# manonkok/Rao-Blackwellized-SLAM-smoothing

Hardware: AMD Instinct MI355X
Metric: particle-steps/s (filter) + smoother wall-clock, N=65k T=3k (higher is better)
Workload: dtype f64

## Files before the change

include/rbpf.h:

```cpp
#ifndef RBPF_H_
#define RBPF_H_

#include <stddef.h>
#include <stdint.h>

#ifdef __cplusplus
extern "C" {
#endif

#define RBPF_ABI_VERSION 9

typedef enum {
  RBPF_OK = 0,
  RBPF_ERR_INVALID_ARG = 1,
  RBPF_ERR_UNSUPPORTED = 2,
  RBPF_ERR_HIP = 3,
  RBPF_ERR_NO_DEVICE = 4,
  RBPF_ERR_OUT_OF_MEMORY = 5,
  RBPF_ERR_CHOL_FAILED = 6,
  RBPF_ERR_STATE = 7,
  RBPF_ERR_CALLBACK = 8
} rbpf_status;

typedef enum {
// ... 221 lines not shown

int rbpf_philox_fill(uint64_t seed, int32_t k_iter, int32_t N_P, int32_t N_T, int32_t n_w,
                     double* U, double* Z, double* Ufin);
int rbpf_meas_model(const rbpf_model* model, int32_t n_nonlin, int32_t n_pred, const double* xn,
                    double* dy);
int rbpf_dyn_model(const rbpf_model* model, int32_t n_nonlin, int32_t n_w, int32_t n_odo,
                   int32_t n_p, const double* xn, const double* odo, double dt, const double* Q,
                   const double* z, double* xn_next);
int rbpf_dyn_res_norm(const rbpf_model* model, int32_t n_nonlin, int32_t n_w, int32_t n_odo,
                      int32_t n_p, const double* xnk_t, const double* xn, const double* odo,
                      double dt, const double* Q, double* e_dyn);
int rbpf_sample(int32_t N, const double* w, int32_t n_draws, const double* u, int32_t* ind);
int rbpf_jacobian_phi3d(const rbpf_model* model, int32_t n_p, const double* x,
                        const double* lower, const double* upper, double* J);
int rbpf_chol_weights(int32_t M, int32_t batch, const double* S, const double* e, double jitter,
                      int32_t variant, int32_t reps, double* logw, int32_t* status, double* ms);
int32_t rbpf_chol_refresh_resolve(int32_t model_kind, int32_t n_lin, int32_t n_y, int32_t requested);
int rbpf_chol_sweep_probe(int32_t n, int32_t d, int32_t batch, const double* L, const double* U, const double* V,
                          const double* eta, int32_t reps, double* L_out, double* logw, int32_t* status, double* ms);
int rbpf_ext_pack_whiten_probe(int32_t dy_layout, int32_t rows, int32_t d, int32_t n, const double* dy_host,
                               const double* W_host, int32_t fused, double* G_host);
int rbpf_quat_helpers(int32_t op, int32_t n, const double* in, double* out);
int rbpf_probe_wave_reduce(const double* in, double* out);

typedef struct {
  int32_t struct_size;
  int32_t m_basis;
  const int32_t* NN;
  double L[3];
  const double* mean;
  const double* V;
  double sigma2;
  const double* var_table;
} rbpf_loc_map;

typedef struct {
  int32_t struct_size;
  int32_t N_P, N_T;
  int32_t x0_cols;
  int32_t q_pages;
  int32_t dt_len;
  int32_t odo_ld;
  const double* odometry;
  const double* y;
  const double* x0_nonlin;
  const double* Q;
// ... 71 lines not shown
```

rao-blackwellized-slam-smoothing_amd/_ffi.py:

```python
from __future__ import annotations

import ctypes as C
import importlib.util
import os
import sys

from . import _build

c_double_p = C.POINTER(C.c_double)
c_int32_p = C.POINTER(C.c_int32)

RBPF_OK = 0
RBPF_ERR_INVALID_ARG = 1
RBPF_ERR_UNSUPPORTED = 2
RBPF_ERR_HIP = 3
RBPF_ERR_NO_DEVICE = 4
RBPF_ERR_OUT_OF_MEMORY = 5
RBPF_ERR_CHOL_FAILED = 6
RBPF_ERR_STATE = 7
RBPF_ERR_CALLBACK = 8

RBPF_MODEL_DENSE_MAG_6D = 1
RBPF_MODEL_DENSE_RADIO_2DH = 2
RBPF_MODEL_SPARSE_VISUAL_2D = 3
# ... 100 lines not shown
class rbpf_ekf_problem(_SizedStructure):
    _fields_ = [("struct_size", C.c_int32), ("n_runs", C.c_int32), ("N_T", C.c_int32), ("q_pages", C.c_int32),
                ("dt_len", C.c_int32), ("odo_ld", C.c_int32), ("keep_P", C.c_int32), ("models", C.POINTER(C.POINTER(rbpf_model))),
                ("odometry", c_double_p), ("y", c_double_p), ("x0", c_double_p), ("q0", c_double_p), ("P0", c_double_p),
                ("R", c_double_p), ("LL", c_double_p), ("Q", c_double_p), ("dt", c_double_p)]


class rbpf_ekf_out(_SizedStructure):
    _fields_ = [("struct_size", C.c_int32), ("reserved", C.c_int32), ("xf_traj", c_double_p), ("qnb_traj", c_double_p),
                ("Pf", c_double_p)]


ABI_STRUCTS = [rbpf_model, rbpf_problem, rbpf_rng, rbpf_options, rbpf_filter_out, rbpf_smoother_out, rbpf_timing, rbpf_callbacks, rbpf_view,
               rbpf_loc_map, rbpf_loc_problem, rbpf_loc_out, rbpf_ekf_problem, rbpf_ekf_out]

EXPORTS = [
    "rbpf_abi_version", "rbpf_abi_sizeof", "rbpf_status_string", "rbpf_last_error", "rbpf_device_count", "rbpf_device_bytes_live",
    "rbpf_particle_filter", "rbpf_particle_smoother", "rbpf_particle_smoother_device",
    "rbpf_filter_create", "rbpf_filter_workspace_bytes", "rbpf_filter_advance", "rbpf_filter_reset", "rbpf_sync",
    "rbpf_filter_finish", "rbpf_filter_tell", "rbpf_filter_schedule", "rbpf_filter_one_launch_flushes", "rbpf_filter_resample_fallbacks", "rbpf_plan_refresh", "rbpf_chol_refresh_resolve", "rbpf_shard_smoother_refresh_reserve", "rbpf_shard_xn_traj", "rbpf_filter_ancestors", "rbpf_filter_step_external", "rbpf_filter_external_layout", "rbpf_filter_ancestors_device",
    "rbpf_filter_step_device", "rbpf_filter_set_device_callbacks",
    "rbpf_filter_sparse_gathered_device", "rbpf_filter_step_sparse_device", "rbpf_filter_sparse_yhattraj", "rbpf_timing_enable", "rbpf_timing_read", "rbpf_destroy",
    "rbpf_philox_fill", "rbpf_meas_model", "rbpf_dyn_model", "rbpf_dyn_res_norm", "rbpf_sample",
    "rbpf_jacobian_phi3d", "rbpf_chol_weights", "rbpf_chol_sweep_probe", "rbpf_ext_pack_whiten_probe", "rbpf_quat_helpers", "rbpf_probe_wave_reduce",
    "rbpf_shard_create", "rbpf_shard_views_get", "rbpf_shard_normalise_search", "rbpf_shard_pack", "rbpf_shard_step",
    "rbpf_shard_trajectories", "rbpf_shard_plan", "rbpf_shard_plan_read", "rbpf_shard_normalise_plan",
    "rbpf_stream_get", "rbpf_shard_set_async", "rbpf_shard_finish", "rbpf_shard_set_ancestors",
    "rbpf_shard_smoother_create", "rbpf_shard_smoother_views_get", "rbpf_shard_smoother_begin",
    "rbpf_shard_smoother_normalise", "rbpf_shard_smoother_anc_weights", "rbpf_shard_smoother_anc_sample",
    "rbpf_shard_smoother_refresh_begin", "rbpf_shard_smoother_refresh_pack", "rbpf_shard_smoother_refresh_end",
    "rbpf_shard_smoother_step", "rbpf_shard_smoother_end",
    "rbpf_particle_filter_localization", "rbpf_loc_create", "rbpf_loc_advance", "rbpf_loc_finish", "rbpf_loc_workspace_bytes",
    "rbpf_loc_predict", "rbpf_loc_dyn_model",
    "rbpf_loc_backward_simulate", "rbpf_loc_history", "rbpf_loc_backward_workspace_bytes", "rbpf_loc_backward_step",
    "rbpf_ekf_dense", "rbpf_ekf_workspace_bytes",
]

ABI_VERSION = 9
_lib = None


class RBPFError(RuntimeError):
    def __init__(self, status, msg):
        super().__init__(f"rbpf status {status}: {msg}")
        self.status = status


# ... 65 lines not shown
    lib.rbpf_filter_step_sparse_device.argtypes = [C.c_void_p, C.c_void_p, C.c_void_p, C.c_int32, C.c_void_p, C.c_int32]
    lib.rbpf_filter_sparse_yhattraj.argtypes = [C.c_void_p, c_double_p]
    lib.rbpf_stream_get.argtypes = [C.c_void_p, C.POINTER(C.c_void_p)]
    lib.rbpf_timing_enable.argtypes = [C.c_void_p, C.c_int32]
    lib.rbpf_timing_read.argtypes = [C.c_void_p, C.POINTER(rbpf_timing), C.c_int32]
    lib.rbpf_destroy.argtypes = [C.c_void_p]
    lib.rbpf_philox_fill.argtypes = [C.c_uint64, C.c_int32, C.c_int32, C.c_int32, C.c_int32, c_double_p, c_double_p,
                                     c_double_p]
    lib.rbpf_meas_model.argtypes = [C.POINTER(rbpf_model), C.c_int32, C.c_int32, c_double_p, c_double_p]
    lib.rbpf_dyn_model.argtypes = [C.POINTER(rbpf_model), C.c_int32, C.c_int32, C.c_int32, C.c_int32, c_double_p,
                                   c_double_p, C.c_double, c_double_p, c_double_p, c_double_p]
    lib.rbpf_dyn_res_norm.argtypes = [C.POINTER(rbpf_model), C.c_int32, C.c_int32, C.c_int32, C.c_int32, c_double_p,
                                      c_double_p, c_double_p, C.c_double, c_double_p, c_double_p]
    lib.rbpf_sample.argtypes = [C.c_int32, c_double_p, C.c_int32, c_double_p, c_int32_p]
    lib.rbpf_jacobian_phi3d.argtypes = [C.POINTER(rbpf_model), C.c_int32, c_double_p, c_double_p, c_double_p,
                                        c_double_p]
    lib.rbpf_chol_weights.argtypes = [C.c_int32, C.c_int32, c_double_p, c_double_p, C.c_double, C.c_int32, C.c_int32,
                                      c_double_p, c_int32_p, c_double_p]
    lib.rbpf_chol_sweep_probe.argtypes = [C.c_int32, C.c_int32, C.c_int32, c_double_p, c_double_p, c_double_p, c_double_p, C.c_int32,
                                          c_double_p, c_double_p, c_int32_p, c_double_p]
    lib.rbpf_ext_pack_whiten_probe.argtypes = [C.c_int32, C.c_int32, C.c_int32, C.c_int32, c_double_p, c_double_p, C.c_int32,
                                               c_double_p]
    lib.rbpf_quat_helpers.argtypes = [C.c_int32, C.c_int32, c_double_p, c_double_p]
    lib.rbpf_chol_refresh_resolve.argtypes = [C.c_int32, C.c_int32, C.c_int32, C.c_int32]
    lib.rbpf_chol_refresh_resolve.restype = C.c_int32
    lib.rbpf_particle_filter_localization.argtypes = [C.POINTER(rbpf_loc_map), C.POINTER(rbpf_loc_problem), C.POINTER(rbpf_rng),
                                                      C.POINTER(rbpf_options), C.POINTER(rbpf_loc_out)]
    lib.rbpf_loc_create.argtypes = [C.POINTER(rbpf_loc_map), C.POINTER(rbpf_loc_problem), C.POINTER(rbpf_rng),
                                    C.POINTER(rbpf_options), C.POINTER(C.c_void_p)]
    lib.rbpf_loc_advance.argtypes = [C.c_void_p, C.c_int32]
    lib.rbpf_loc_finish.argtypes = [C.c_void_p, C.POINTER(rbpf_loc_out)]
    lib.rbpf_loc_workspace_bytes.argtypes = [C.POINTER(rbpf_loc_map), C.POINTER(rbpf_loc_problem), C.POINTER(rbpf_options),
                                             C.POINTER(C.c_size_t)]
    lib.rbpf_loc_predict.argtypes = [C.POINTER(rbpf_loc_map), C.c_int32, c_double_p, c_double_p, c_double_p, C.c_int32, c_double_p]
    lib.rbpf_loc_dyn_model.argtypes = [C.c_int32, c_double_p, c_double_p, C.c_double, c_double_p, c_double_p, c_double_p]
    lib.rbpf_loc_backward_simulate.argtypes = [C.c_void_p, C.c_int32, c_double_p, C.c_uint64, c_double_p, c_int32_p, c_double_p]
    lib.rbpf_loc_history.argtypes = [C.c_void_p, c_double_p]
    lib.rbpf_loc_backward_workspace_bytes.argtypes = [C.c_int32, C.c_int32, C.c_int32, C.POINTER(C.c_size_t)]
    lib.rbpf_loc_backward_step.argtypes = [C.c_int32, C.c_int32, c_double_p, c_double_p, c_double_p, c_double_p, C.c_double, c_double_p,
                                           c_double_p, c_int32_p, c_double_p, C.c_int32, c_double_p]
    lib.rbpf_ekf_dense.argtypes = [C.POINTER(rbpf_ekf_problem), C.POINTER(rbpf_options), C.POINTER(rbpf_ekf_out)]
    lib.rbpf_ekf_workspace_bytes.argtypes = [C.POINTER(rbpf_ekf_problem), C.POINTER(rbpf_options), C.POINTER(C.c_size_t)]
    _lib = lib
    return lib


# ... 6 lines not shown
```

rao-blackwellized-slam-smoothing_amd/csrc/rbpf_api.hip:

```cpp
#include "../../include/rbpf.h"
#include "rbpf_internal.hpp"
#include "rbpf_ctx.hpp"
#include "rbpf_sparse.hpp"

#include <cmath>
#include <cstdio>
#include <cstdlib>
#include <cstring>
#include <string>
#include <vector>

namespace rbpf {

thread_local std::string g_last_error;

void set_error(const std::string& s) { g_last_error = s; }

int hip_fail(hipError_t e, const char* what, const char* file, int line) {
  char buf[512];
  snprintf(buf, sizeof(buf), "%s failed: %s (%s:%d)", what, hipGetErrorString(e), file, line);
  g_last_error = buf;
  (void)hipGetLastError();
  return (e == hipErrorOutOfMemory) ? RBPF_ERR_OUT_OF_MEMORY : RBPF_ERR_HIP;
}
// ... 334 lines not shown
  c->lazy_depth = (!sparse && c->opt.lazy_depth >= 2) ? std::min(c->opt.lazy_depth, smoother ? 3 : ((c->lay.sym && c->lay.CH64 == 8 && !c->fp32) ? (int)kMaxSets : (int)kMaxSetsFull)) : 1;
  {
    const bool can = !ex && c->lazy_depth >= 2 && (!smoother || c->opt.inplace > 0);
    if (c->opt.inplace > 0 && !can) { set_error("inplace=1 needs lazy_depth >= 2 and an unsharded session"); return RBPF_ERR_UNSUPPORTED; }
    c->inplace = c->opt.inplace > 0;
    if (c->opt.inplace == 0 && can) {
      size_t fr = 0, tot = 0;
      HIPCHK(hipMemGetInfo(&fr, &tot));
      const size_t two = 2 * c->bank_cap * (L.szT + L.szB) * (c->fp32 ? sizeof(float) : sizeof(double));
      c->inplace = (double)two > 0.85 * (double)fr;
    }
  }
  for (int b = 0; b < 2; ++b) {
    if (b == 1 && c->inplace) { c->Pt[1] = c->Pt[0]; c->Pb[1] = c->Pb[0]; }
    else {
      RB_TRY(c->pool.alloc(&c->Pt[b], c->fp32 ? (c->bank_cap * L.szT + 1) / 2 : c->bank_cap * L.szT));
      RB_TRY(c->pool.alloc(&c->Pb[b], c->fp32 ? (c->bank_cap * L.szB + 1) / 2 : c->bank_cap * L.szB));
    }
    RB_TRY(c->pool.alloc(&c->F[b], c->bank_cap * 2 * d * L.ldx));
    RB_TRY(c->pool.alloc(&c->xl[b], c->bank_cap * L.ldx));
    HIPCHK(hipMemsetAsync(c->F[b], 0, c->bank_cap * 2 * d * L.ldx * sizeof(double), c->stream));
    HIPCHK(hipMemsetAsync(c->xl[b], 0, c->bank_cap * L.ldx * sizeof(double), c->stream));
  }
  if (c->inplace) RB_TRY(c->pool.alloc(&c->d_ip, (size_t)8 * N));
  c->share_inplace = c->inplace && c->lazy_depth >= 2 && !ex && layout_shares_flush(c->lay);
  if (const char* e = tuning_env("RBPF_SHARE_INPLACE")) c->share_inplace = c->share_inplace && atoi(e) != 0;
  if (c->share_inplace) {
    RB_TRY(c->pool.alloc(&c->d_share_writers, 1));
    HIPCHK(hipMemset(c->d_share_writers, 0, sizeof(unsigned long long)));
  }
  c->share_flush = c->lazy_depth >= 2 && !c->inplace && !ex && layout_shares_flush(c->lay);
  if (const size_t sd = sym_strip_doubles(c->lay, d + (smoother ? 1 : 0))) {
    RB_TRY(c->pool.alloc(&c->d_strip_ws, (size_t)N * sd));
    c->strip_ws_stride = sd;
  }
  if (c->share_flush) {
    RB_TRY(c->pool.alloc(&c->d_share, (size_t)3 * N));
    RB_TRY(c->pool.alloc(&c->d_share_writers, 1));
    HIPCHK(hipMemset(c->d_share_writers, 0, sizeof(unsigned long long)));
  }
  if (c->lazy_depth >= 2) {
    if (!L.sym && (L.CH < 1 || L.CPL < 1 || L.CPL > 2)) { set_error("lazy_depth >= 2 needs 128 <= nLin with at most two row chunks per wave (full-square storage; block-lower storage, options.storage = 2, takes nLin 384..511)"); return RBPF_ERR_UNSUPPORTED; }
    if (!L.sym && step_lds_bytes(c->mdl, c->lay, smoother ? 1 : 0, c->lazy_depth) > 160 * 1024) { set_error("lazy_depth too large for the LDS plan"); return RBPF_ERR_UNSUPPORTED; }
    if (L.sym && step_sym_lds_bytes(c->mdl, c->lay, c->lazy_depth, 1, smoother ? 1 : 0) > 160 * 1024) { set_error("lazy_depth too large for the LDS plan"); return RBPF_ERR_UNSUPPORTED; }
    for (int b = 0; b <= c->lazy_depth; ++b) {
      RB_TRY(c->pool.alloc(&c->Fb[b], (size_t)(N + 1) * 2 * d * L.ldx));
      HIPCHK(hipMemsetAsync(c->Fb[b], 0, (size_t)(N + 1) * 2 * d * L.ldx * sizeof(double), c->stream));
// ... 1204 lines not shown
int rbpf_quat_helpers(int32_t op, int32_t n, const double* in, double* out) {
  if (!have_device()) { set_error("no HIP device"); return RBPF_ERR_NO_DEVICE; }
  if (op < 0 || op > 8 || n < 1 || !in || !out) { set_error("bad argument"); return RBPF_ERR_INVALID_ARG; }
  static const int nin_of[9] = {3, 3, 4, 4, 4, 4, 4, 4, 3}, nout_of[9] = {4, 4, 3, 3, 16, 16, 4, 9, 9};
  DevicePool tmp; double *di = nullptr, *dout = nullptr;
  RB_TRY(tmp.upload(&di, in, (size_t)n * nin_of[op])); RB_TRY(tmp.alloc(&dout, (size_t)n * nout_of[op]));
  HIPCHK(launch_quat_helpers(op, n, di, dout, 0));
  HIPCHK(hipDeviceSynchronize());
  HIPCHK(hipMemcpy(out, dout, (size_t)n * nout_of[op] * 8, hipMemcpyDeviceToHost));
  return RBPF_OK;
}

int rbpf_probe_wave_reduce(const double* in, double* out) {
  if (!have_device()) { set_error("no HIP device"); return RBPF_ERR_NO_DEVICE; }
  if (!in || !out) { set_error("bad argument"); return RBPF_ERR_INVALID_ARG; }
  DevicePool tmp; double *di = nullptr, *dout = nullptr;
  RB_TRY(tmp.upload(&di, in, 256)); RB_TRY(tmp.alloc(&dout, 4));
  HIPCHK(launch_probe_wave_reduce(di, dout, 0));
  HIPCHK(hipDeviceSynchronize());
  HIPCHK(hipMemcpy(out, dout, 4 * 8, hipMemcpyDeviceToHost));
  return RBPF_OK;
}

int rbpf_jacobian_phi3d(const rbpf_model* model, int32_t n_p, const double* x, const double* lower, const double* upper, double* J) {
  if (!have_device()) { set_error("no HIP device"); return RBPF_ERR_NO_DEVICE; }
  if (!model || model->kind != RBPF_MODEL_DENSE_MAG_6D || !x || !lower || !upper || !J || n_p < 1) { set_error("bad argument"); return RBPF_ERR_INVALID_ARG; }
  ModelDev M; DevicePool tmp; double *dx = nullptr, *dlo = nullptr, *dup = nullptr, *dj = nullptr;
  RB_TRY(model_for_helpers(model, 7, 6, 7, M, tmp));
  RB_TRY(tmp.upload(&dx, x, (size_t)3 * n_p)); RB_TRY(tmp.upload(&dlo, lower, 3)); RB_TRY(tmp.upload(&dup, upper, 3)); RB_TRY(tmp.alloc(&dj, (size_t)9 * M.m * n_p));
  HIPCHK(launch_jacobian_phi3d(M, n_p, dx, dlo, dup, dj, 0));
  HIPCHK(hipDeviceSynchronize());
  HIPCHK(hipMemcpy(J, dj, (size_t)9 * M.m * n_p * 8, hipMemcpyDeviceToHost));
  return RBPF_OK;
}

}
```

rao-blackwellized-slam-smoothing_amd/csrc/rbpf_internal.hpp:

```cpp
#pragma once
#include <hip/hip_runtime.h>
#include <stdint.h>
#include <stddef.h>
#include <stdlib.h>
#include <atomic>

namespace rbpf {

inline hipError_t lds_opt_in(const void* kernel, int bytes, std::atomic<uint64_t>& done) {
  int dev = 0;
  hipError_t e = hipGetDevice(&dev);
  if (e != hipSuccess) return e;
  const uint64_t bit = 1ull << (dev & 63);
  if (dev < 64 && (done.load(std::memory_order_acquire) & bit)) return hipSuccess;
  e = hipFuncSetAttribute(kernel, hipFuncAttributeMaxDynamicSharedMemorySize, bytes);
  if (e != hipSuccess) return e;
  if (dev < 64) done.fetch_or(bit, std::memory_order_release);
  return hipSuccess;
}

#ifdef RBPF_TUNING
inline const char* tuning_env(const char* key) { return getenv(key); }
#else
inline const char* tuning_env(const char*) { return nullptr; }
// ... 115 lines not shown
  const double* xn;
  double* traj_max;
  double* traj_mean;
  int* iw_max;
  double* lse_out;
  int parallel_scan = 0;
};

struct SearchArgs {
  int N, n_draw, t;
  int slot0 = 0;
  int u_is_scalar = 0;
  const double* wc;
  int rng_mode; int k_iter;
  const double* U;
  unsigned long long seed;
  int* ai;
  int* overflow;
  int scan_depth = 0;
  int approx = 0;
  int* ambiguous = nullptr;
  const double* w = nullptr;
  double* wc_exact = nullptr;
};

size_t step_lds_bytes(const ModelDev& m, const Layout& lay, int extra = 0, int n_sets = 1);
bool step_use_blocked(const ModelDev& m, const Layout& lay, int extra, int n_sets);
Layout make_layout(int n, int d);
Layout make_layout_low_regs(int n, int d);
Layout make_layout_sym(int n, int d, int fp32 = 0);
bool sym_supported(int n, int d);
size_t sym_strip_doubles(const Layout& lay, int d);
size_t step_sym_lds_bytes(const ModelDev& m, const Layout& lay, int n_sets, int write_base, int extra = 0);
hipError_t launch_step_sym(const StepArgs& a, hipStream_t s);
bool step_sym_shared_one_launch(const StepArgs& a);
hipError_t launch_step_sym_shared(const StepArgs& a, hipStream_t s);
hipError_t launch_probe_wave_reduce(const double* in, double* out, hipStream_t s);

hipError_t launch_propagate(const StepArgs& a, hipStream_t s);
hipError_t launch_step(const StepArgs& a, hipStream_t s);
hipError_t launch_step_wide_d2(const StepArgs& a, hipStream_t s);
hipError_t launch_step_wide_d4(const StepArgs& a, hipStream_t s);
hipError_t launch_step_wide_d5(const StepArgs& a, hipStream_t s);
hipError_t launch_step_wide_d6(const StepArgs& a, hipStream_t s);
hipError_t launch_step_wide_d7(const StepArgs& a, hipStream_t s);
hipError_t launch_step_wide_d8(const StepArgs& a, hipStream_t s);
hipError_t launch_normalise_scan(const NormArgs& a, hipStream_t s);
hipError_t launch_search(const SearchArgs& a, hipStream_t s);
hipError_t launch_cumsum(int N, const double* w, double* wc, hipStream_t s);
hipError_t launch_normalise_resample(const NormArgs& a, const SearchArgs& sa, int* order, int* counts, hipStream_t s,
                                     const int* remap = nullptr);
hipError_t launch_order_large(int n_slots, int range, const int* key, const int* remap, int* order, int* counts, hipStream_t s);
hipError_t launch_order(int n_slots, int range, const int* key, int* order, int* counts, hipStream_t s, const int* remap = nullptr);
hipError_t launch_inplace_plan(int N, const int* order, const int* ai, const int* base, int* dst, int* phase,
                               int* scratch, hipStream_t s);
hipError_t launch_share_inplace_plan(int N, const int* order, const int* ai, const int* base, int* dst, int* phase, int* scratch,
                                     unsigned long long* writers, hipStream_t s);
hipError_t launch_share_plan(int N, int nkeys, const int* ai, int* lead, int* dst, int* phase, unsigned long long* writers, hipStream_t s);
size_t resample_scratch_doubles(int N);
hipError_t launch_resample_pipeline(const NormArgs& nm, const SearchArgs* sa, int* order, int* counts, const int* remap,
                                    double* scratch, hipStream_t s);
hipError_t launch_resample_lse(int N, const double* scratch, double* out, hipStream_t s);
constexpr int kMaxParticles = 1024 * 1024;
constexpr int kSingleWgResampleMaxN = 8192;
hipError_t launch_resample_fixup(const SearchArgs& a, hipStream_t s);

hipError_t launch_pack_P(const Layout& lay, const double* P_colmajor, size_t src_stride, double* Pt,
                         double* Pb, int count, hipStream_t s, int fp32 = 0);
hipError_t launch_unpack_P(const Layout& lay, int d, const double* Pt, const double* Pb, const double* F,
                           const int* index, int count, double* P_colmajor, hipStream_t s, int fp32 = 0);
hipError_t launch_unpack_P_sets(const Layout& lay, int d, const double* Pt, const double* Pb, int n_sets,
                                const double* const* fset, const int* const* fidx, const int* base, const int* index,
                                int count, double* P_colmajor, hipStream_t s, int fp32 = 0);
hipError_t launch_weighted_mean_xl(int N, int n, int ldx, const double* xl, const double* w, double* out,
// ... 35 lines not shown
```

rao-blackwellized-slam-smoothing_amd/csrc/rbpf_kernels.hip:

```cpp
#include "rbpf_internal.hpp"
#include "rbpf_device.hpp"
#include "rbpf_model_dev.hpp"

#include <cstdlib>

#include "rbpf_step_full.hpp"

namespace rbpf {

Layout make_layout_low_regs(int n, int d) {
  Layout L = make_layout(n, d);
  if (L.CH == 2) { L.RS = 2; L.CS = 2; L.CPL = L.CH / L.RS; }
  return L;
}

#ifndef RBPF_KB_THRESHOLD_KB
#define RBPF_KB_THRESHOLD_KB 72
#endif
bool step_use_blocked(const ModelDev& m, const Layout& lay, int extra, int n_sets) {
  if (n_sets < 1 || lay.mc == 0 || lay.CPL < 1 || lay.CPL > 2 || lay.CH != lay.CPL * lay.RS || lay.RS * lay.CS != kWaves) return false;
  return (size_t)lds_plan(lay.n, m.d, extra, n_sets, lay.ldx, lay.CS, lay.mc, m.ktot, 0).total * sizeof(double) > (size_t)RBPF_KB_THRESHOLD_KB * 1024;
}

size_t step_lds_bytes(const ModelDev& m, const Layout& lay, int extra, int n_sets) {
// ... 521 lines not shown
}

hipError_t launch_order(int n_slots, int range, const int* key, int* order, int* counts, hipStream_t s, const int* remap) {
  if (range > kSingleWgResampleMaxN) return launch_order_large(n_slots, range, key, remap, order, counts, s);
  hipLaunchKernelGGL(order_kernel, dim3(1), dim3(kNormThreads), 0, s, n_slots, range, key, order, counts, remap);
  return hipGetLastError();
}

__global__ __launch_bounds__(kNormThreads) void cumsum_kernel(int N, const double* __restrict__ w,
                                                              double* __restrict__ wc) {
  __shared__ double sbuf[kScanChunk];
  __shared__ double sbuf2[kScanChunk];
  __shared__ double scarry;
  strict_cumsum_block(N, w, wc, sbuf, sbuf2, &scarry);
}

hipError_t launch_cumsum(int N, const double* w, double* wc, hipStream_t s) {
  hipLaunchKernelGGL(cumsum_kernel, dim3(1), dim3(kNormThreads), 0, s, N, w, wc);
  return hipGetLastError();
}

__global__ void search_kernel(const SearchArgs a) {
  const int i0 = blockIdx.x * blockDim.x + threadIdx.x;
  if (i0 >= a.n_draw) return;
  const int i = a.slot0 + i0;
  const double u = (a.rng_mode == 0) ? a.U[a.u_is_scalar ? 0 : i] : philox_resample_uniform(a.seed, i, a.t, a.k_iter);
  int lo = 0, hi = a.N;
  while (lo < hi) {
    const int mid = (lo + hi) >> 1;
    if (a.wc[mid] < u) lo = mid + 1; else hi = mid;
  }
  if (a.approx) {
    const double S = a.scan_depth > 0 ? (double)a.scan_depth : (double)((a.N + kNormThreads - 1) / kNormThreads) + 32.0;
    bool amb = false;
    if (lo < a.N) { const double p = a.wc[lo]; amb |= fabs(p - u) <= 1.7e-16 * ((double)lo + S) * fabs(p); }
    if (lo > 0) { const double p = a.wc[lo - 1]; amb |= fabs(p - u) <= 1.7e-16 * ((double)lo + S) * fabs(p); }
    if (amb) atomicAdd(a.ambiguous, 1);
  }
  if (lo >= a.N) { lo = a.N - 1; if (a.overflow) atomicAdd(a.overflow, 1); }
  a.ai[i] = lo;
}

__global__ __launch_bounds__(kNormThreads) void resample_fixup_kernel(const SearchArgs a) {
  __shared__ double sbuf[kScanChunk];
  __shared__ double sbuf2[kScanChunk];
  __shared__ double scarry;
// ... 479 lines not shown
```

rao-blackwellized-slam-smoothing_amd/csrc/rbpf_resample.hip:

```cpp
#include "rbpf_internal.hpp"
#include "rbpf_device.hpp"

namespace rbpf {

constexpr int kRB = 1024;

__device__ inline double blk_sum(double v, double* sred) {
  const int lane = threadIdx.x & 63, wave = threadIdx.x >> 6;
  v = wave_sum(v);
  __syncthreads();
  if (lane == 0) sred[wave] = v;
  __syncthreads();
  double s = sred[0];
  for (int w = 1; w < kRB / 64; ++w) s += sred[w];
  return s;
}

__device__ inline double blk_max(double v, double* sred) {
  const int lane = threadIdx.x & 63, wave = threadIdx.x >> 6;
#pragma unroll
  for (int off = 32; off > 0; off >>= 1) v = fmax(v, __shfl_xor(v, off, 64));
  __syncthreads();
  if (lane == 0) sred[wave] = v;
  __syncthreads();
  double s = sred[0];
  for (int w = 1; w < kRB / 64; ++w) s = fmax(s, sred[w]);
  return s;
}

__global__ __launch_bounds__(kRB) void rs_max_kernel(int N, const double* __restrict__ logw, double* __restrict__ pmax) {
  __shared__ double sred[16];
  const int i = blockIdx.x * kRB + threadIdx.x;
  const double m = blk_max(i < N ? logw[i] : -INFINITY, sred);
  if (threadIdx.x == 0) pmax[blockIdx.x] = m;
}

__device__ inline double global_max(const double* pmax, int B, double* sred) {
  double m = -INFINITY;
  for (int b = threadIdx.x; b < B; b += kRB) m = fmax(m, pmax[b]);
  return blk_max(m, sred);
}

__global__ __launch_bounds__(kRB) void rs_sumexp_kernel(int N, int B, const double* __restrict__ logw,
                                                        const double* __restrict__ pmax, double* __restrict__ psum) {
  __shared__ double sred[16];
  const double c = global_max(pmax, B, sred);
  const int i = blockIdx.x * kRB + threadIdx.x;
  const double s = blk_sum(i < N ? exp(logw[i] - c) : 0.0, sred);
  if (threadIdx.x == 0) psum[blockIdx.x] = s;
}

__global__ __launch_bounds__(kRB) void rs_weights_kernel(NormArgs a, int B, const double* __restrict__ pmax,
                                                         const double* __restrict__ psum, double* __restrict__ btot,
                                                         double* __restrict__ bparts ) {
  __shared__ double sred[16];
  __shared__ int sidx[16];
  __shared__ double sbc;
  const int tid = threadIdx.x, lane = tid & 63, wave = tid >> 6, N = a.N;
  const double c = global_max(pmax, B, sred);
  if (tid == 0) { double t = 0.0; for (int b = 0; b < B; ++b) t += psum[b]; sbc = c + log(t); }
  __syncthreads();
  const double lse = sbc;
  const int i = blockIdx.x * kRB + tid;
  const double wi = (i < N) ? exp(a.logw[i] - lse) : 0.0;
  if (i < N) a.w[i] = wi;
  double bw = (i < N) ? wi : -1.0;
  int bi = (i < N) ? i : 0x7fffffff;
#pragma unroll
  for (int off = 32; off > 0; off >>= 1) {
    const double ow = __shfl_xor(bw, off, 64);
    const int oi = __shfl_xor(bi, off, 64);
    if (ow > bw || (ow == bw && oi < bi)) { bw = ow; bi = oi; }
  }
  __syncthreads();
  if (lane == 0) { sred[wave] = bw; sidx[wave] = bi; }
  __syncthreads();
  if (tid == 0) {
    double gw = sred[0]; int gi = sidx[0];
    for (int w = 1; w < kRB / 64; ++w) if (sred[w] > gw || (sred[w] == gw && sidx[w] < gi)) { gw = sred[w]; gi = sidx[w]; }
    bparts[blockIdx.x * 10 + 0] = gw;
    bparts[blockIdx.x * 10 + 1] = (double)gi;
  }
  for (int cix = 0; cix < a.nN; ++cix) {
// ... 11 lines not shown
  __syncthreads();
  double woff = 0.0;
  for (int w = 0; w < wave; ++w) woff += sred[w];
  const double lp = woff + inc;
  if (i < N) a.wc[i] = lp;
  if (tid == kRB - 1) btot[blockIdx.x] = lp;
}

__global__ __launch_bounds__(kRB) void rs_offsets_kernel(NormArgs a, int B, const double* __restrict__ btot,
                                                         const double* __restrict__ bparts) {
  __shared__ double sb[1024];
  __shared__ double sp[16][10];
  __shared__ double soff;
  const int tid = threadIdx.x, N = a.N;
  for (int b = tid; b < B; b += kRB) sb[b] = btot[b];
  __syncthreads();
  if (tid == 0) { double t = 0.0; for (int b = 0; b < (int)blockIdx.x; ++b) t += sb[b]; soff = t; }
  __syncthreads();
  const int i = blockIdx.x * kRB + tid;
  if (i < N && blockIdx.x > 0) a.wc[i] = soff + a.wc[i];
  if (blockIdx.x == 0) {
    if (tid < 2 + a.nN) {
      const int q = tid;
      if (q >= 2) {
        double t = 0.0;
        for (int b = 0; b < B; ++b) t += bparts[b * 10 + q];
        sp[0][q] = t;
      }
    }
    if (tid == 0) {
      double gw = bparts[0]; int gi = (int)bparts[1];
      for (int b = 1; b < B; ++b) { const double w = bparts[b * 10]; const int ix = (int)bparts[b * 10 + 1]; if (w > gw || (w == gw && ix < gi)) { gw = w; gi = ix; } }
      if (gi < 0 || gi >= N) gi = 0;
      *a.iw_max = gi;
      sp[1][0] = (double)gi;
    }
    __syncthreads();
    if (tid >= 2 && tid < 2 + a.nN) {
      const int cix = tid - 2, gi = (int)sp[1][0];
      if (a.traj_mean) a.traj_mean[cix] = sp[0][tid];
      if (a.traj_max) a.traj_max[cix] = a.xn[(size_t)cix * N + gi];
    }
  }
}

__global__ void rs_hist_kernel(int N, const int* __restrict__ key, const int* __restrict__ remap, int* __restrict__ counts) {
  const int i = blockIdx.x * blockDim.x + threadIdx.x;
  if (i < N) atomicAdd(&counts[remap ? remap[key[i]] : key[i]], 1);
}

__global__ __launch_bounds__(kRB) void rs_scan_kernel(int N, int* __restrict__ counts) {
  __shared__ int swave[kRB / 64];
  const int tid = threadIdx.x, lane = tid & 63, wave = tid >> 6;
  const int S = (N + kRB - 1) / kRB;
  const int j0 = min(tid * S, N), j1 = min(j0 + S, N);
  constexpr int NBATCH = 8;
  int tot = 0;
  for (int jb = j0; jb < j1; jb += NBATCH) {
    int v[NBATCH];
#pragma unroll
    for (int k = 0; k < NBATCH; ++k) v[k] = counts[min(jb + k, N - 1)];
#pragma unroll
    for (int k = 0; k < NBATCH; ++k) tot += (jb + k < j1) ? v[k] : 0;
  }
  int inc = tot;
#pragma unroll
  for (int off = 1; off < 64; off <<= 1) { const int o = __shfl_up(inc, off, 64); if (lane >= off) inc += o; }
  if (lane == 63) swave[wave] = inc;
  __syncthreads();
  int run = inc - tot;
  for (int w = 0; w < wave; ++w) run += swave[w];
  for (int jb = j0; jb < j1; jb += NBATCH) {
    int v[NBATCH];
#pragma unroll
    for (int k = 0; k < NBATCH; ++k) v[k] = counts[min(jb + k, N - 1)];
#pragma unroll
    for (int k = 0; k < NBATCH; ++k)
      if (jb + k < j1) { counts[jb + k] = run; run += v[k]; }
  }
}

__global__ void rs_scatter_kernel(int N, const int* __restrict__ key, const int* __restrict__ remap, int* __restrict__ counts,
                                  int* __restrict__ order) {
  const int i = blockIdx.x * blockDim.x + threadIdx.x;
  if (i < N) order[atomicAdd(&counts[remap ? remap[key[i]] : key[i]], 1)] = i;
}

size_t resample_scratch_doubles(int N) { return (size_t)13 * ((N + kRB - 1) / kRB) + 16; }

hipError_t launch_resample_pipeline(const NormArgs& nm, const SearchArgs* sa, int* order, int* counts, const int* remap,
                                    double* scratch, hipStream_t s) {
  const int N = nm.N, B = (N + kRB - 1) / kRB;
  double* pmax = scratch; double* psum = pmax + B; double* btot = psum + B; double* bparts = btot + B;
  hipLaunchKernelGGL(rs_max_kernel, dim3(B), dim3(kRB), 0, s, N, nm.logw, pmax);
  hipLaunchKernelGGL(rs_sumexp_kernel, dim3(B), dim3(kRB), 0, s, N, B, nm.logw, pmax, psum);
  hipLaunchKernelGGL(rs_weights_kernel, dim3(B), dim3(kRB), 0, s, nm, B, pmax, psum, btot, bparts);
  hipLaunchKernelGGL(rs_offsets_kernel, dim3(B), dim3(kRB), 0, s, nm, B, btot, bparts);
  hipError_t e = hipGetLastError();
  if (e != hipSuccess || !sa) return e;
  SearchArgs q = *sa;
  q.scan_depth = B + 32;
  if ((e = launch_search(q, s)) != hipSuccess) return e;
  if (q.approx && (e = launch_resample_fixup(q, s)) != hipSuccess) return e;
  if (order) {
    if ((e = hipMemsetAsync(counts, 0, (size_t)N * sizeof(int), s)) != hipSuccess) return e;
    const int nb = (q.n_draw + 255) / 256;
    hipLaunchKernelGGL(rs_hist_kernel, dim3(nb), dim3(256), 0, s, q.n_draw, q.ai, remap, counts);
    hipLaunchKernelGGL(rs_scan_kernel, dim3(1), dim3(kRB), 0, s, N, counts);
    hipLaunchKernelGGL(rs_scatter_kernel, dim3(nb), dim3(256), 0, s, q.n_draw, q.ai, remap, counts, order);
    e = hipGetLastError();
  }
  return e;
}

__global__ void rs_lse_kernel(int B, const double* __restrict__ pmax, const double* __restrict__ psum, double* __restrict__ out) {
  double c = -INFINITY, t = 0.0;
  for (int b = 0; b < B; ++b) c = fmax(c, pmax[b]);
  for (int b = 0; b < B; ++b) t += psum[b];
  *out = c + log(t);
}

hipError_t launch_resample_lse(int N, const double* scratch, double* out, hipStream_t s) {
  const int B = (N + kRB - 1) / kRB;
  hipLaunchKernelGGL(rs_lse_kernel, dim3(1), dim3(1), 0, s, B, scratch, scratch + B, out);
  return hipGetLastError();
}

hipError_t launch_order_large(int n_slots, int range, const int* key, const int* remap, int* order, int* counts, hipStream_t s) {
  hipError_t e = hipMemsetAsync(counts, 0, (size_t)range * sizeof(int), s);
  if (e != hipSuccess) return e;
  const int nb = (n_slots + 255) / 256;
  hipLaunchKernelGGL(rs_hist_kernel, dim3(nb), dim3(256), 0, s, n_slots, key, remap, counts);
  hipLaunchKernelGGL(rs_scan_kernel, dim3(1), dim3(kRB), 0, s, range, counts);
  hipLaunchKernelGGL(rs_scatter_kernel, dim3(nb), dim3(256), 0, s, n_slots, key, remap, counts, order);
  return hipGetLastError();
}

__global__ void ip_mark_kernel(int N, const int* __restrict__ ai, const int* __restrict__ base, int* __restrict__ has,
                               int* __restrict__ nzp) {
  const int i = blockIdx.x * blockDim.x + threadIdx.x;
  if (i < N) { const int s = base[ai[i]]; has[s] = 1; nzp[s] = 1; }
}

__global__ void ip_free_kernel(int N, const int* __restrict__ has, const int* __restrict__ nzp, int* __restrict__ freelist) {
  const int f = blockIdx.x * blockDim.x + threadIdx.x;
  if (f < N && !has[f]) freelist[f - nzp[f]] = f;
}

__global__ void ip_assign_kernel(int N, const int* __restrict__ order, const int* __restrict__ ai, const int* __restrict__ base,
                                 const int* __restrict__ nzp, const int* __restrict__ freelist, int* __restrict__ dst,
                                 int* __restrict__ phase) {
  const int b = blockIdx.x * blockDim.x + threadIdx.x;
  if (b >= N) return;
  const int i = order[b];
  const int s = base[ai[i]];
  const int prev = (b > 0) ? base[ai[order[b - 1]]] : -1;
  const bool first = (s != prev);
  dst[i] = first ? s : freelist[b - nzp[s] - 1];
// ... 53 lines not shown
  const int b = blockIdx.x * blockDim.x + threadIdx.x;
  bool w = false;
  if (b < N) {
    const int i = order[b];
    w = lead[ai[i]] == i;
    if (w) {
      const int s = base[ai[i]];
      const bool first = leadbase[s] == b;
      dst[i] = first ? s : freelist[rank[b]];
      phase[i] = first ? 2 : 1;
    }
  }
  const unsigned long long m = __ballot(w);
  if (writers && (threadIdx.x & 63) == 0 && m) atomicAdd(writers, (unsigned long long)__popcll(m));
}
__global__ void sip_readers_kernel(int N, const int* __restrict__ ai, const int* __restrict__ lead, int* __restrict__ dst, int* __restrict__ phase) {
  const int i = blockIdx.x * blockDim.x + threadIdx.x;
  if (i < N && lead[ai[i]] != i) { dst[i] = dst[lead[ai[i]]]; phase[i] = 0; }
}

hipError_t launch_share_inplace_plan(int N, const int* order, const int* ai, const int* base, int* dst, int* phase, int* scratch,
                                     unsigned long long* writers, hipStream_t s) {
  int* lead = scratch; int* leadbase = scratch + N; int* has = scratch + 2 * (size_t)N; int* nzp = scratch + 3 * (size_t)N;
  int* freelist = scratch + 4 * (size_t)N; int* flag = scratch + 5 * (size_t)N;
  const int nb = (N + 255) / 256;
  hipLaunchKernelGGL(sip_fill_kernel, dim3(nb), dim3(256), 0, s, N, lead, leadbase, has, nzp);
  hipLaunchKernelGGL(sip_mark_kernel, dim3(nb), dim3(256), 0, s, N, ai, base, lead, has, nzp);
  hipLaunchKernelGGL(rs_scan_kernel, dim3(1), dim3(kRB), 0, s, N, nzp);
  hipLaunchKernelGGL(ip_free_kernel, dim3(nb), dim3(256), 0, s, N, has, nzp, freelist);
  hipLaunchKernelGGL(sip_first_kernel, dim3(nb), dim3(256), 0, s, N, order, ai, base, lead, leadbase);
  hipLaunchKernelGGL(sip_flag_kernel, dim3(nb), dim3(256), 0, s, N, order, ai, base, lead, leadbase, flag);
  hipLaunchKernelGGL(rs_scan_kernel, dim3(1), dim3(kRB), 0, s, N, flag);
  hipLaunchKernelGGL(sip_writers_kernel, dim3(nb), dim3(256), 0, s, N, order, ai, base, lead, leadbase, flag, freelist, dst, phase, writers);
  hipLaunchKernelGGL(sip_readers_kernel, dim3(nb), dim3(256), 0, s, N, ai, lead, dst, phase);
  return hipGetLastError();
}

hipError_t launch_inplace_plan(int N, const int* order, const int* ai, const int* base, int* dst, int* phase, int* scratch,
                               hipStream_t s) {
  int* has = scratch; int* nzp = scratch + N; int* freelist = scratch + 2 * (size_t)N;
  hipError_t e = hipMemsetAsync(scratch, 0, (size_t)2 * N * sizeof(int), s);
  if (e != hipSuccess) return e;
  const int nb = (N + 255) / 256;
  hipLaunchKernelGGL(ip_mark_kernel, dim3(nb), dim3(256), 0, s, N, ai, base, has, nzp);
  hipLaunchKernelGGL(rs_scan_kernel, dim3(1), dim3(kRB), 0, s, N, nzp);
  hipLaunchKernelGGL(ip_free_kernel, dim3(nb), dim3(256), 0, s, N, has, nzp, freelist);
  hipLaunchKernelGGL(ip_assign_kernel, dim3(nb), dim3(256), 0, s, N, order, ai, base, nzp, freelist, dst, phase);
  return hipGetLastError();
}

}
```

Before: 5.949 million.

## Replace single-block integer scans with multi-block scan in resample ordering

Swaps the single-workgroup serial-chunk exclusive scan used in counting-sort ordering and in-place plan building for a multi-block scan. Each block scans its own slice, and block offsets are then folded in, either by a separate add pass or directly inside the scatter kernel. The counts memset is folded into the search kernel, and the tid-0 serial reductions over block partials are batched so loads can be issued ahead of the adds. This is meant to remove a one-block serial bottleneck at N=65k, at the cost of extra launches, per-block recomputation of offsets, and a larger scratch buffer.

Result: no change. 5.928 million (-0.4%).

```diff
diff --git a/include/rbpf.h b/include/rbpf.h
--- a/include/rbpf.h
+++ b/include/rbpf.h
@@ -267,6 +267,8 @@
                                const double* W_host, int32_t fused, double* G_host);
 int rbpf_quat_helpers(int32_t op, int32_t n, const double* in, double* out);
 int rbpf_probe_wave_reduce(const double* in, double* out);
+int rbpf_order_scan_probe(int32_t n_slots, int32_t range, const int32_t* key, int32_t n_remap, const int32_t* remap, int32_t* order,
+                          int32_t* scan);
 
 typedef struct {
   int32_t struct_size;
diff --git a/rao-blackwellized-slam-smoothing_amd/_ffi.py b/rao-blackwellized-slam-smoothing_amd/_ffi.py
--- a/rao-blackwellized-slam-smoothing_amd/_ffi.py
+++ b/rao-blackwellized-slam-smoothing_amd/_ffi.py
@@ -146,7 +146,7 @@
     "rbpf_filter_step_device", "rbpf_filter_set_device_callbacks",
     "rbpf_filter_sparse_gathered_device", "rbpf_filter_step_sparse_device", "rbpf_filter_sparse_yhattraj", "rbpf_timing_enable", "rbpf_timing_read", "rbpf_destroy",
     "rbpf_philox_fill", "rbpf_meas_model", "rbpf_dyn_model", "rbpf_dyn_res_norm", "rbpf_sample",
-    "rbpf_jacobian_phi3d", "rbpf_chol_weights", "rbpf_chol_sweep_probe", "rbpf_ext_pack_whiten_probe", "rbpf_quat_helpers", "rbpf_probe_wave_reduce",
+    "rbpf_jacobian_phi3d", "rbpf_chol_weights", "rbpf_chol_sweep_probe", "rbpf_ext_pack_whiten_probe", "rbpf_quat_helpers", "rbpf_probe_wave_reduce", "rbpf_order_scan_probe",
     "rbpf_shard_create", "rbpf_shard_views_get", "rbpf_shard_normalise_search", "rbpf_shard_pack", "rbpf_shard_step",
     "rbpf_shard_trajectories", "rbpf_shard_plan", "rbpf_shard_plan_read", "rbpf_shard_normalise_plan",
     "rbpf_stream_get", "rbpf_shard_set_async", "rbpf_shard_finish", "rbpf_shard_set_ancestors",
@@ -258,6 +258,7 @@
     lib.rbpf_ext_pack_whiten_probe.argtypes = [C.c_int32, C.c_int32, C.c_int32, C.c_int32, c_double_p, c_double_p, C.c_int32,
                                                c_double_p]
     lib.rbpf_quat_helpers.argtypes = [C.c_int32, C.c_int32, c_double_p, c_double_p]
+    lib.rbpf_order_scan_probe.argtypes = [C.c_int32, C.c_int32, c_int32_p, C.c_int32, c_int32_p, c_int32_p, c_int32_p]
     lib.rbpf_chol_refresh_resolve.argtypes = [C.c_int32, C.c_int32, C.c_int32, C.c_int32]
     lib.rbpf_chol_refresh_resolve.restype = C.c_int32
     lib.rbpf_particle_filter_localization.argtypes = [C.POINTER(rbpf_loc_map), C.POINTER(rbpf_loc_problem), C.POINTER(rbpf_rng),
diff --git a/rao-blackwellized-slam-smoothing_amd/csrc/rbpf_api.hip b/rao-blackwellized-slam-smoothing_amd/csrc/rbpf_api.hip
--- a/rao-blackwellized-slam-smoothing_amd/csrc/rbpf_api.hip
+++ b/rao-blackwellized-slam-smoothing_amd/csrc/rbpf_api.hip
@@ -380,7 +380,7 @@
     HIPCHK(hipMemsetAsync(c->F[b], 0, c->bank_cap * 2 * d * L.ldx * sizeof(double), c->stream));
     HIPCHK(hipMemsetAsync(c->xl[b], 0, c->bank_cap * L.ldx * sizeof(double), c->stream));
   }
-  if (c->inplace) RB_TRY(c->pool.alloc(&c->d_ip, (size_t)8 * N));
+  if (c->inplace) RB_TRY(c->pool.alloc(&c->d_ip, (size_t)8 * N + scan_scratch_ints((size_t)N)));
   c->share_inplace = c->inplace && c->lazy_depth >= 2 && !ex && layout_shares_flush(c->lay);
   if (const char* e = tuning_env("RBPF_SHARE_INPLACE")) c->share_inplace = c->share_inplace && atoi(e) != 0;
   if (c->share_inplace) {
@@ -1631,6 +1631,31 @@
   return RBPF_OK;
 }
 
+int rbpf_order_scan_probe(int32_t n_slots, int32_t range, const int32_t* key, int32_t n_remap, const int32_t* remap, int32_t* order,
+                          int32_t* scan) {
+  if (!have_device()) { set_error("no HIP device"); return RBPF_ERR_NO_DEVICE; }
+  if (range < 1 || range > kMaxParticles || (!key && !scan) || (key && (!order || n_slots < 1 || n_slots > kMaxParticles)) ||
+      (remap && n_remap < 1)) { set_error("bad argument"); return RBPF_ERR_INVALID_ARG; }
+  const int nkeys = remap ? n_remap : range;
+  for (int i = 0; key && i < n_slots; ++i)
+    if (key[i] < 0 || key[i] >= nkeys || (remap && (remap[key[i]] < 0 || remap[key[i]] >= range))) { set_error("key out of range"); return RBPF_ERR_INVALID_ARG; }
+  DevicePool tmp; int *dkey = nullptr, *dremap = nullptr, *dorder = nullptr, *dcounts = nullptr, *dscan = nullptr, *dtot = nullptr;
+  if (key) {
+    RB_TRY(tmp.upload(&dkey, key, (size_t)n_slots)); RB_TRY(tmp.alloc(&dorder, (size_t)n_slots));
+    if (remap) RB_TRY(tmp.upload(&dremap, remap, (size_t)n_remap));
+    RB_TRY(tmp.alloc(&dcounts, (size_t)range + scan_scratch_ints((size_t)range)));
+    HIPCHK(launch_order_large(n_slots, range, dkey, dremap, dorder, dcounts, 0));
+  }
+  if (scan) {
+    RB_TRY(tmp.upload(&dscan, scan, (size_t)range)); RB_TRY(tmp.alloc(&dtot, scan_scratch_ints((size_t)range)));
+    HIPCHK(launch_scan_ints(range, dscan, dtot, 0));
+  }
+  HIPCHK(hipDeviceSynchronize());
+  if (key) HIPCHK(hipMemcpy(order, dorder, (size_t)n_slots * 4, hipMemcpyDeviceToHost));
+  if (scan) HIPCHK(hipMemcpy(scan, dscan, (size_t)range * 4, hipMemcpyDeviceToHost));
+  return RBPF_OK;
+}
+
 int rbpf_jacobian_phi3d(const rbpf_model* model, int32_t n_p, const double* x, const double* lower, const double* upper, double* J) {
   if (!have_device()) { set_error("no HIP device"); return RBPF_ERR_NO_DEVICE; }
   if (!model || model->kind != RBPF_MODEL_DENSE_MAG_6D || !x || !lower || !upper || !J || n_p < 1) { set_error("bad argument"); return RBPF_ERR_INVALID_ARG; }
diff --git a/rao-blackwellized-slam-smoothing_amd/csrc/rbpf_internal.hpp b/rao-blackwellized-slam-smoothing_amd/csrc/rbpf_internal.hpp
--- a/rao-blackwellized-slam-smoothing_amd/csrc/rbpf_internal.hpp
+++ b/rao-blackwellized-slam-smoothing_amd/csrc/rbpf_internal.hpp
@@ -161,6 +161,8 @@
   int* ambiguous = nullptr;
   const double* w = nullptr;
   double* wc_exact = nullptr;
+  int* zero = nullptr;
+  int n_zero = 0;
 };
 
 size_t step_lds_bytes(const ModelDev& m, const Layout& lay, int extra = 0, int n_sets = 1);
@@ -189,6 +191,8 @@
 hipError_t launch_cumsum(int N, const double* w, double* wc, hipStream_t s);
 hipError_t launch_normalise_resample(const NormArgs& a, const SearchArgs& sa, int* order, int* counts, hipStream_t s,
                                      const int* remap = nullptr);
+constexpr size_t scan_scratch_ints(size_t n) { return (n + 1023) / 1024; }
+hipError_t launch_scan_ints(int n, int* data, int* btot, hipStream_t s);
 hipError_t launch_order_large(int n_slots, int range, const int* key, const int* remap, int* order, int* counts, hipStream_t s);
 hipError_t launch_order(int n_slots, int range, const int* key, int* order, int* counts, hipStream_t s, const int* remap = nullptr);
 hipError_t launch_inplace_plan(int N, const int* order, const int* ai, const int* base, int* dst, int* phase,
diff --git a/rao-blackwellized-slam-smoothing_amd/csrc/rbpf_kernels.hip b/rao-blackwellized-slam-smoothing_amd/csrc/rbpf_kernels.hip
--- a/rao-blackwellized-slam-smoothing_amd/csrc/rbpf_kernels.hip
+++ b/rao-blackwellized-slam-smoothing_amd/csrc/rbpf_kernels.hip
@@ -567,6 +567,8 @@
 
 __global__ void search_kernel(const SearchArgs a) {
   const int i0 = blockIdx.x * blockDim.x + threadIdx.x;
+  if (a.zero)
+    for (int j = i0; j < a.n_zero; j += gridDim.x * blockDim.x) a.zero[j] = 0;
   if (i0 >= a.n_draw) return;
   const int i = a.slot0 + i0;
   const double u = (a.rng_mode == 0) ? a.U[a.u_is_scalar ? 0 : i] : philox_resample_uniform(a.seed, i, a.t, a.k_iter);
diff --git a/rao-blackwellized-slam-smoothing_amd/csrc/rbpf_resample.hip b/rao-blackwellized-slam-smoothing_amd/csrc/rbpf_resample.hip
--- a/rao-blackwellized-slam-smoothing_amd/csrc/rbpf_resample.hip
+++ b/rao-blackwellized-slam-smoothing_amd/csrc/rbpf_resample.hip
@@ -14,6 +14,19 @@
   double s = sred[0];
   for (int w = 1; w < kRB / 64; ++w) s += sred[w];
   return s;
+}
+
+constexpr int kSumBatch = 16;
+__device__ inline double ordered_sum(const double* __restrict__ x, int n, int stride) {
+  double t = 0.0;
+  for (int b0 = 0; b0 < n; b0 += kSumBatch) {
+    double v[kSumBatch];
+#pragma unroll
+    for (int k = 0; k < kSumBatch; ++k) v[k] = x[(size_t)min(b0 + k, n - 1) * stride];
+#pragma unroll
+    for (int k = 0; k < kSumBatch; ++k) if (b0 + k < n) t += v[k];
+  }
+  return t;
 }
 
 __device__ inline double blk_max(double v, double* sred) {
@@ -58,7 +71,7 @@
   __shared__ double sbc;
   const int tid = threadIdx.x, lane = tid & 63, wave = tid >> 6, N = a.N;
   const double c = global_max(pmax, B, sred);
-  if (tid == 0) { double t = 0.0; for (int b = 0; b < B; ++b) t += psum[b]; sbc = c + log(t); }
+  if (tid == 0) sbc = c + log(ordered_sum(psum, B, 1));
   __syncthreads();
   const double lse = sbc;
   const int i = blockIdx.x * kRB + tid;
@@ -116,15 +129,20 @@
   if (blockIdx.x == 0) {
     if (tid < 2 + a.nN) {
       const int q = tid;
-      if (q >= 2) {
-        double t = 0.0;
-        for (int b = 0; b < B; ++b) t += bparts[b * 10 + q];
-        sp[0][q] = t;
-      }
+      if (q >= 2) sp[0][q] = ordered_sum(bparts + q, B, 10);
     }
     if (tid == 0) {
       double gw = bparts[0]; int gi = (int)bparts[1];
-      for (int b = 1; b < B; ++b) { const double w = bparts[b * 10]; const int ix = (int)bparts[b * 10 + 1]; if (w > gw || (w == gw && ix < gi)) { gw = w; gi = ix; } }
+      for (int b0 = 1; b0 < B; b0 += kSumBatch) {
+        double vw[kSumBatch], vi[kSumBatch];
+#pragma unroll
+        for (int k = 0; k < kSumBatch; ++k) { const int b = min(b0 + k, B - 1); vw[k] = bparts[b * 10]; vi[k] = bparts[b * 10 + 1]; }
+#pragma unroll
+        for (int k = 0; k < kSumBatch; ++k) {
+          const double w = vw[k]; const int ix = (int)vi[k];
+          if (b0 + k < B && (w > gw || (w == gw && ix < gi))) { gw = w; gi = ix; }
+        }
+      }
       if (gi < 0 || gi >= N) gi = 0;
       *a.iw_max = gi;
       sp[1][0] = (double)gi;
@@ -138,46 +156,85 @@
   }
 }
 
-__global__ void rs_hist_kernel(int N, const int* __restrict__ key, const int* __restrict__ remap, int* __restrict__ counts) {
-  const int i = blockIdx.x * blockDim.x + threadIdx.x;
-  if (i < N) atomicAdd(&counts[remap ? remap[key[i]] : key[i]], 1);
-}
-
-__global__ __launch_bounds__(kRB) void rs_scan_kernel(int N, int* __restrict__ counts) {
+constexpr int kMaxScanBlocks = kMaxParticles / kRB;
+
+__global__ __launch_bounds__(kRB) void rs_blockscan_kernel(int n, int* __restrict__ data, int* __restrict__ btot) {
   __shared__ int swave[kRB / 64];
   const int tid = threadIdx.x, lane = tid & 63, wave = tid >> 6;
-  const int S = (N + kRB - 1) / kRB;
-  const int j0 = min(tid * S, N), j1 = min(j0 + S, N);
-  constexpr int NBATCH = 8;
-  int tot = 0;
-  for (int jb = j0; jb < j1; jb += NBATCH) {
-    int v[NBATCH];
-#pragma unroll
-    for (int k = 0; k < NBATCH; ++k) v[k] = counts[min(jb + k, N - 1)];
-#pragma unroll
-    for (int k = 0; k < NBATCH; ++k) tot += (jb + k < j1) ? v[k] : 0;
-  }
-  int inc = tot;
+  const int i = blockIdx.x * kRB + tid;
+  const int v = (i < n) ? data[i] : 0;
+  int inc = v;
 #pragma unroll
   for (int off = 1; off < 64; off <<= 1) { const int o = __shfl_up(inc, off, 64); if (lane >= off) inc += o; }
   if (lane == 63) swave[wave] = inc;
   __syncthreads();
-  int run = inc - tot;
+  int run = inc - v;
   for (int w = 0; w < wave; ++w) run += swave[w];
-  for (int jb = j0; jb < j1; jb += NBATCH) {
-    int v[NBATCH];
-#pragma unroll
-    for (int k = 0; k < NBATCH; ++k) v[k] = counts[min(jb + k, N - 1)];
-#pragma unroll
-    for (int k = 0; k < NBATCH; ++k)
-      if (jb + k < j1) { counts[jb + k] = run; run += v[k]; }
-  }
-}
-
-__global__ void rs_scatter_kernel(int N, const int* __restrict__ key, const int* __restrict__ remap, int* __restrict__ counts,
-                                  int* __restrict__ order) {
-  const int i = blockIdx.x * blockDim.x + threadIdx.x;
-  if (i < N) order[atomicAdd(&counts[remap ? remap[key[i]] : key[i]], 1)] = i;
+  if (i < n) data[i] = run;
+  if (tid == kRB - 1) btot[blockIdx.x] = run + v;
+}
+
+__device__ inline void rs_block_offsets(int B, const int* __restrict__ btot, int* sboff, int* swave) {
+  const int tid = threadIdx.x, lane = tid & 63, wave = tid >> 6, nwaves = blockDim.x >> 6;
+  int carry = 0;
+  for (int b0 = 0; b0 < B; b0 += blockDim.x) {
+    const int b = b0 + tid;
+    const int v = (b < B) ? btot[b] : 0;
+    int inc = v;
+#pragma unroll
+    for (int off = 1; off < 64; off <<= 1) { const int o = __shfl_up(inc, off, 64); if (lane >= off) inc += o; }
+    __syncthreads();
+    if (lane == 63) swave[wave] = inc;
+    __syncthreads();
+    int run = carry + inc - v;
+    for (int w = 0; w < wave; ++w) run += swave[w];
+    if (b < B) sboff[b] = run;
+    for (int w = 0; w < nwaves; ++w) carry += swave[w];
+  }
+  __syncthreads();
+}
+
+__global__ __launch_bounds__(kRB) void rs_addoffsets_kernel(int n, int B, int* __restrict__ data, const int* __restrict__ btot) {
+  __shared__ int sboff[kMaxScanBlocks];
+  __shared__ int swave[kRB / 64];
+  rs_block_offsets(B, btot, sboff, swave);
+  const int i = blockIdx.x * kRB + threadIdx.x;
+  if (i < n) data[i] += sboff[blockIdx.x];
+}
+
+hipError_t launch_scan_ints(int n, int* data, int* btot, hipStream_t s) {
+  const int B = (n + kRB - 1) / kRB;
+  if (n < 1 || B > kMaxScanBlocks) return hipErrorInvalidValue;
+  hipLaunchKernelGGL(rs_blockscan_kernel, dim3(B), dim3(kRB), 0, s, n, data, btot);
+  if (B > 1) hipLaunchKernelGGL(rs_addoffsets_kernel, dim3(B), dim3(kRB), 0, s, n, B, data, btot);
+  return hipGetLastError();
+}
+
+__global__ void rs_hist_kernel(int N, const int* __restrict__ key, const int* __restrict__ remap, int* __restrict__ counts) {
+  const int i = blockIdx.x * blockDim.x + threadIdx.x;
+  if (i < N) atomicAdd(&counts[remap ? remap[key[i]] : key[i]], 1);
+}
+
+__global__ __launch_bounds__(256) void rs_scatter_kernel(int N, int B, const int* __restrict__ key, const int* __restrict__ remap,
+                                                         int* __restrict__ counts, const int* __restrict__ btot, int* __restrict__ order) {
+  __shared__ int sboff[kMaxScanBlocks];
+  __shared__ int swave[4];
+  rs_block_offsets(B, btot, sboff, swave);
+  const int i = blockIdx.x * blockDim.x + threadIdx.x;
+  if (i < N) {
+    const int k = remap ? remap[key[i]] : key[i];
+    order[sboff[k / kRB] + atomicAdd(&counts[k], 1)] = i;
+  }
+}
+
+static hipError_t launch_order_chain(int n_slots, int range, const int* key, const int* remap, int* order, int* counts, hipStream_t s) {
+  const int nb = (n_slots + 255) / 256, B = (range + kRB - 1) / kRB;
+  if (n_slots < 1 || range < 1 || B > kMaxScanBlocks) return hipErrorInvalidValue;
+  int* btot = counts + range;
+  hipLaunchKernelGGL(rs_hist_kernel, dim3(nb), dim3(256), 0, s, n_slots, key, remap, counts);
+  hipLaunchKernelGGL(rs_blockscan_kernel, dim3(B), dim3(kRB), 0, s, range, counts, btot);
+  hipLaunchKernelGGL(rs_scatter_kernel, dim3(nb), dim3(256), 0, s, n_slots, B, key, remap, counts, btot, order);
+  return hipGetLastError();
 }
 
 size_t resample_scratch_doubles(int N) { return (size_t)13 * ((N + kRB - 1) / kRB) + 16; }
@@ -194,16 +251,13 @@
   if (e != hipSuccess || !sa) return e;
   SearchArgs q = *sa;
   q.scan_depth = B + 32;
+  if (order) {
+    if (q.n_draw < 1) return hipErrorInvalidValue;
+    q.zero = counts; q.n_zero = N;
+  }
   if ((e = launch_search(q, s)) != hipSuccess) return e;
   if (q.approx && (e = launch_resample_fixup(q, s)) != hipSuccess) return e;
-  if (order) {
-    if ((e = hipMemsetAsync(counts, 0, (size_t)N * sizeof(int), s)) != hipSuccess) return e;
-    const int nb = (q.n_draw + 255) / 256;
-    hipLaunchKernelGGL(rs_hist_kernel, dim3(nb), dim3(256), 0, s, q.n_draw, q.ai, remap, counts);
-    hipLaunchKernelGGL(rs_scan_kernel, dim3(1), dim3(kRB), 0, s, N, counts);
-    hipLaunchKernelGGL(rs_scatter_kernel, dim3(nb), dim3(256), 0, s, q.n_draw, q.ai, remap, counts, order);
-    e = hipGetLastError();
-  }
+  if (order) e = launch_order_chain(q.n_draw, N, q.ai, remap, order, counts, s);
   return e;
 }
 
@@ -221,13 +275,9 @@
 }
 
 hipError_t launch_order_large(int n_slots, int range, const int* key, const int* remap, int* order, int* counts, hipStream_t s) {
-  hipError_t e = hipMemsetAsync(counts, 0, (size_t)range * sizeof(int), s);
+  const hipError_t e = hipMemsetAsync(counts, 0, (size_t)range * sizeof(int), s);
   if (e != hipSuccess) return e;
-  const int nb = (n_slots + 255) / 256;
-  hipLaunchKernelGGL(rs_hist_kernel, dim3(nb), dim3(256), 0, s, n_slots, key, remap, counts);
-  hipLaunchKernelGGL(rs_scan_kernel, dim3(1), dim3(kRB), 0, s, range, counts);
-  hipLaunchKernelGGL(rs_scatter_kernel, dim3(nb), dim3(256), 0, s, n_slots, key, remap, counts, order);
-  return hipGetLastError();
+  return launch_order_chain(n_slots, range, key, remap, order, counts, s);
 }
 
 __global__ void ip_mark_kernel(int N, const int* __restrict__ ai, const int* __restrict__ base, int* __restrict__ has,
@@ -327,15 +377,16 @@
 hipError_t launch_share_inplace_plan(int N, const int* order, const int* ai, const int* base, int* dst, int* phase, int* scratch,
                                      unsigned long long* writers, hipStream_t s) {
   int* lead = scratch; int* leadbase = scratch + N; int* has = scratch + 2 * (size_t)N; int* nzp = scratch + 3 * (size_t)N;
-  int* freelist = scratch + 4 * (size_t)N; int* flag = scratch + 5 * (size_t)N;
+  int* freelist = scratch + 4 * (size_t)N; int* flag = scratch + 5 * (size_t)N; int* btot = scratch + 6 * (size_t)N;
   const int nb = (N + 255) / 256;
+  hipError_t e;
   hipLaunchKernelGGL(sip_fill_kernel, dim3(nb), dim3(256), 0, s, N, lead, leadbase, has, nzp);
   hipLaunchKernelGGL(sip_mark_kernel, dim3(nb), dim3(256), 0, s, N, ai, base, lead, has, nzp);
-  hipLaunchKernelGGL(rs_scan_kernel, dim3(1), dim3(kRB), 0, s, N, nzp);
+  if ((e = launch_scan_ints(N, nzp, btot, s)) != hipSuccess) return e;
   hipLaunchKernelGGL(ip_free_kernel, dim3(nb), dim3(256), 0, s, N, has, nzp, freelist);
   hipLaunchKernelGGL(sip_first_kernel, dim3(nb), dim3(256), 0, s, N, order, ai, base, lead, leadbase);
   hipLaunchKernelGGL(sip_flag_kernel, dim3(nb), dim3(256), 0, s, N, order, ai, base, lead, leadbase, flag);
-  hipLaunchKernelGGL(rs_scan_kernel, dim3(1), dim3(kRB), 0, s, N, flag);
+  if ((e = launch_scan_ints(N, flag, btot, s)) != hipSuccess) return e;
   hipLaunchKernelGGL(sip_writers_kernel, dim3(nb), dim3(256), 0, s, N, order, ai, base, lead, leadbase, flag, freelist, dst, phase, writers);
   hipLaunchKernelGGL(sip_readers_kernel, dim3(nb), dim3(256), 0, s, N, ai, lead, dst, phase);
   return hipGetLastError();
@@ -343,12 +394,12 @@
 
 hipError_t launch_inplace_plan(int N, const int* order, const int* ai, const int* base, int* dst, int* phase, int* scratch,
                                hipStream_t s) {
-  int* has = scratch; int* nzp = scratch + N; int* freelist = scratch + 2 * (size_t)N;
+  int* has = scratch; int* nzp = scratch + N; int* freelist = scratch + 2 * (size_t)N; int* btot = scratch + 3 * (size_t)N;
   hipError_t e = hipMemsetAsync(scratch, 0, (size_t)2 * N * sizeof(int), s);
   if (e != hipSuccess) return e;
   const int nb = (N + 255) / 256;
   hipLaunchKernelGGL(ip_mark_kernel, dim3(nb), dim3(256), 0, s, N, ai, base, has, nzp);
-  hipLaunchKernelGGL(rs_scan_kernel, dim3(1), dim3(kRB), 0, s, N, nzp);
+  if ((e = launch_scan_ints(N, nzp, btot, s)) != hipSuccess) return e;
   hipLaunchKernelGGL(ip_free_kernel, dim3(nb), dim3(256), 0, s, N, has, nzp, freelist);
   hipLaunchKernelGGL(ip_assign_kernel, dim3(nb), dim3(256), 0, s, N, order, ai, base, nzp, freelist, dst, phase);
   return hipGetLastError();
```
